# arkworks-rs/accumulation

Measured on NVIDIA B200. Metric: Pallas MSM Mpts/s @2^20, higher is better.
Workload: dtype u32x8 (255-bit Montgomery)

## Files before the change

accumulation_b200/csrc/accmsm.cu:

```cuda
#include <algorithm>
#include <chrono>
#include <cstdint>
#include <cstdio>
#include <cstdlib>
#include <cstring>
#include <functional>
#include <mutex>
#include <string>
#include <unordered_map>
#include <vector>

#include "../../include/accmsm.h"
#include "msm.cuh"
#include "sort.cuh"
#include "vec.cuh"
#include "ipa.cuh"
#include "wire.cuh"
#include "hostfp.hpp"

using namespace accmsm;

namespace {

enum Stage { ST_H2D = 0, ST_DIGITS, ST_SCAN, ST_SCATTER, ST_ACCUMULATE, ST_FIXUP, ST_REDUCE, ST_FINISH, ST_D2H, ST_VEC, ST_VEC_D2H, ST_COUNT };
// ... 30 lines not shown
void ipa_session_free(IpaSession *s);
struct CsrSet;
void csr_set_free(CsrSet *c);

struct GroupWorker;
struct GroupKey;
struct GroupCsr;

struct accmsm_ctx {
    std::vector<accmsm_ctx *> kids;
    std::vector<GroupWorker *> workers;
    std::unordered_map<uint64_t, GroupKey *> gkeys;
    std::unordered_map<uint64_t, GroupCsr *> gcsrs;
    std::unordered_map<uint64_t, struct GroupIpaSession *> gsessions;
    std::vector<char> peer_ok;
    std::vector<char> peer_read;
    void *d_gather = nullptr;
    size_t min_shard = size_t(1) << 16;
    int device = 0;
    int sm_count = 0;
    cudaStream_t stream = nullptr;
    std::mutex mu;
    std::string last_error;
    std::unordered_map<uint64_t, Bases> bases;
    std::unordered_map<uint64_t, struct IpaSession *> ipa_sessions;
    std::vector<struct IpaSession *> ipa_free;
    std::unordered_map<uint64_t, struct CsrSet *> csr_sets;
    std::vector<std::pair<void *, size_t>> vec_cache;
    uint64_t next_handle = 1;
    int window_bits = 0;
    uint64_t launches = 0;
    int acc_ctas_per_sm[2] = {0, 0};

    DevBuf<uint32_t> digits, hist, offsets, cursor, entries, cta_ids, tile_sums, tile_offs;
    DevBuf<xyzz_t> buckets, red_sum[2], red_wsum[2], cta_parts, partial;
    DevBuf<uint8_t> scalars, misc;
    DevBuf<uint2> sort_pairs;
    DevBuf<uint32_t> sort_tile_count, sort_part_count, sort_part_offs;
    int segments_override = 0;
    int seg0_pct = 25;
    std::vector<int> seg_pcts;
    bool no_coop_precompute = false;
    bool trace = false;
    std::vector<std::pair<std::string, cudaEvent_t>> trace_ev;
    std::vector<double> trace_host_us;
    int sort_lb_override = 0;
    DevBuf<uint8_t> oneshot_inf, ipa_tabs;
    bool no_ipa_tabs = false;
    bool no_coop_finish = false;
    DevBuf<affine_t> oneshot_xy, pair_pts[2];
    DevBuf<uint32_t> pair_off[2];
    DevBuf<uint8_t> pair_pref, pair_kinds, pair_tfac, pair_ctot, pair_cfac;
    int affine_rounds_override = -1;
    DevBuf<xyzz_t> fold_partial;
    DevBuf<uint32_t> fold_flag;
    int ipa_fold_rounds = 5, ipa_fold_min_log = 11;
    int fk_small_c = 0;
    xyzz_t *d_out_raw = nullptr;
    int out_curve = 0;
    uint64_t *h_out = nullptr;
    void *h_stage = nullptr;
    size_t stage_cap = 0;
    cudaEvent_t stage_done = nullptr;
    bool stage_busy = false;
    std::vector<cudaEvent_t> chunk_events;
    cudaStream_t copy_stream = nullptr;
    cudaStream_t aux_stream = nullptr;
    cudaEvent_t aux_fork = nullptr, aux_join = nullptr;
// ... 148 lines not shown
            *storage_cap = records;
        }
        table = *storage;
    } else {
        CU(ctx, cudaMalloc(&table, records * sizeof(affine_t)));
    }
    if (B.n <= PRECOMPUTE_COOP_MAX && !ctx->no_coop_precompute) {
        uint32_t groups = (uint32_t)((B.n + 31) / 32);
        if (B.curve == 0) k_precompute_coop<0><<<groups, 128, 0, ctx->stream>>>(B.d_xy, (uint32_t)B.n, c, nwin, table);
        else k_precompute_coop<1><<<groups, 128, 0, ctx->stream>>>(B.d_xy, (uint32_t)B.n, c, nwin, table);
    } else {
        uint32_t blocks = (uint32_t)((B.n + 127) / 128);
        if (B.curve == 0) k_precompute<0><<<blocks, 128, 0, ctx->stream>>>(B.d_xy, (uint32_t)B.n, c, nwin, table);
        else k_precompute<1><<<blocks, 128, 0, ctx->stream>>>(B.d_xy, (uint32_t)B.n, c, nwin, table);
    }
    ctx->launches++;
    if (!storage) {
        cudaError_t e = cudaStreamSynchronize(ctx->stream);
        if (e != cudaSuccess) { cudaFree(table); CU(ctx, e); }
    }
    B.d_table = table; B.pre_c = c; B.pre_nwin = nwin;
    return ACCMSM_OK;
}

bool use_table(const accmsm_ctx *ctx, const Bases &B, size_t n) {
    (void)n;
    if (!B.d_table) return false;
    return !ctx->window_bits || (uint32_t)ctx->window_bits == B.pre_c;
}

constexpr uint32_t ACC_WARP_MAX_KEYS = 8192;
constexpr size_t ACC_WARP_MAX_ENTRIES = 1u << 17;

#ifndef RED_L0_BLK
#define RED_L0_BLK 32
#endif

struct MsmJobs {
    uint32_t njobs = 1;
    size_t offset[MAX_JOBS] = {0};
    uint32_t tail_base = NONE_ID;
    uint32_t map_log_h = NONE_ID;
    MsmJobs() {}
    explicit MsmJobs(size_t off) { offset[0] = off; }
};

MsmShape make_shape(const accmsm_ctx *ctx, const Bases &B, const MsmJobs &jobs, size_t n, size_t n_for_c) {
    MsmShape sh;
    sh.n = (uint32_t)n;
    sh.njobs = jobs.njobs;
    sh.tail_base = jobs.tail_base;
    sh.map_log_h = jobs.map_log_h;
    for (int j = 0; j < MAX_JOBS; j++) sh.job_off[j] = j < (int)jobs.njobs ? (uint32_t)jobs.offset[j] : 0u;
    if (use_table(ctx, B, n)) {
        sh.c = B.pre_c;
        sh.nwin = B.pre_nwin;
        sh.nb = 1u << (sh.c - 1);
        sh.sets_per_job = 1;
        sh.hist_stride = 0;
        sh.ent_stride = (uint32_t)B.n;
    } else {
        sh.c = pick_window_bits(ctx, n_for_c);
        sh.nwin = (256 + sh.c - 1) / sh.c;
        sh.nb = 1u << (sh.c - 1);
        sh.sets_per_job = sh.nwin;
        sh.hist_stride = sh.nb;
        sh.ent_stride = 0;
    }
    sh.nkeys = sh.njobs * sh.sets_per_job * sh.nb;
    return sh;
// ... 107 lines not shown
        mark(ctx, ST_FIXUP, st);
    } else {
        const uint32_t *acc_offsets = ctx->offsets.p, *acc_entries = ctx->entries.p;
        const affine_t *acc_points = points;
        size_t acc_bound = n_entries;
        int rounds = into ? 0 : affine_rounds(ctx, sh, n_entries);
        for (int r = 0; r < rounds; r++) {
            const size_t out_bound = (acc_bound + sh.nkeys) / 2 + 1;
            CU(ctx, ctx->pair_off[r & 1].ensure(sh.nkeys + 1));
            CU(ctx, ctx->pair_pts[r & 1].ensure(out_bound));
            k_pair_counts<<<(sh.nkeys + 255) / 256, 256, 0, st>>>(acc_offsets, sh.nkeys, ctx->hist.p);
            ctx->launches++;
            { int src2 = launch_scan(ctx, ctx->hist.p, sh.nkeys, ctx->pair_off[r & 1].p, nullptr, st); if (src2) return src2; }
            uint32_t pgrid = (uint32_t)((out_bound + (size_t)PAIR_THREADS * PAIR_B - 1) / ((size_t)PAIR_THREADS * PAIR_B));
            CU(ctx, ctx->pair_pref.ensure(out_bound * 32));
            CU(ctx, ctx->pair_kinds.ensure(out_bound));
            CU(ctx, ctx->pair_tfac.ensure((size_t)pgrid * PAIR_THREADS * 32));
            CU(ctx, ctx->pair_ctot.ensure((size_t)pgrid * 32));
            CU(ctx, ctx->pair_cfac.ensure((size_t)pgrid * 32));
            const uint32_t *oin = acc_offsets, *oout = ctx->pair_off[r & 1].p;
            affine_t *pout = ctx->pair_pts[r & 1].p;
            if (r == 0) {
                k_pair_fwd<CURVE, true><<<pgrid, PAIR_THREADS, 0, st>>>(oin, oout, sh.nkeys, ctx->entries.p, points, ctx->pair_pref.p, ctx->pair_kinds.p, ctx->pair_tfac.p, ctx->pair_ctot.p);
                k_pair_mid<CURVE><<<1, PAIR_MID_THREADS, 0, st>>>(oout, sh.nkeys, ctx->pair_ctot.p, ctx->pair_cfac.p);
                k_pair_bwd<CURVE, true><<<pgrid, PAIR_THREADS, 0, st>>>(oin, oout, sh.nkeys, ctx->entries.p, points, ctx->pair_pref.p, ctx->pair_kinds.p, ctx->pair_tfac.p, ctx->pair_cfac.p, pout);
            } else {
                k_pair_fwd<CURVE, false><<<pgrid, PAIR_THREADS, 0, st>>>(oin, oout, sh.nkeys, nullptr, acc_points, ctx->pair_pref.p, ctx->pair_kinds.p, ctx->pair_tfac.p, ctx->pair_ctot.p);
                k_pair_mid<CURVE><<<1, PAIR_MID_THREADS, 0, st>>>(oout, sh.nkeys, ctx->pair_ctot.p, ctx->pair_cfac.p);
                k_pair_bwd<CURVE, false><<<pgrid, PAIR_THREADS, 0, st>>>(oin, oout, sh.nkeys, nullptr, acc_points, ctx->pair_pref.p, ctx->pair_kinds.p, ctx->pair_tfac.p, ctx->pair_cfac.p, pout);
            }
            ctx->launches += 3;
            acc_offsets = ctx->pair_off[r & 1].p; acc_entries = nullptr; acc_points = ctx->pair_pts[r & 1].p; acc_bound = out_bound;
        }
        int per_sm = ctx->acc_ctas_per_sm[CURVE];
        uint32_t gmax = (uint32_t)(ctx->sm_count * per_sm);
        uint32_t want = (uint32_t)((acc_bound + (size_t)ACC_THREADS * 8 - 1) / ((size_t)ACC_THREADS * 8));
        uint32_t grid = std::max(1u, std::min(gmax, want));
        CU(ctx, ctx->cta_ids.ensure(2 * grid));
        CU(ctx, ctx->cta_parts.ensure(2 * grid));
        size_t smem = 2 * ACC_THREADS * (sizeof(xyzz_t) + sizeof(uint32_t));
        if (into) k_accumulate<CURVE, true><<<grid, ACC_THREADS, smem, st>>>(acc_offsets, sh.nkeys, acc_entries, acc_points, ctx->buckets.p,
                                                                              ctx->cta_ids.p, ctx->cta_parts.p);
        else k_accumulate<CURVE, false><<<grid, ACC_THREADS, smem, st>>>(acc_offsets, sh.nkeys, acc_entries, acc_points, ctx->buckets.p,
                                                                          ctx->cta_ids.p, ctx->cta_parts.p);
        mark(ctx, ST_FIXUP, st);
        trace_point(ctx, st, "  k_accumulate done");
        uint32_t ns = 2 * grid;
        if (ns > (uint32_t)(FIX_THREADS * FIX_PER_T)) return fail_arg(ctx, "msm: accumulate grid exceeds the fix-up kernel's slots");
        size_t smem2 = ns * (sizeof(xyzz_t) + sizeof(uint32_t));
        cudaStream_t fx = fixup_aside ? aux_begin(ctx, st) : st;
        k_fixup<CURVE><<<1, FIX_THREADS, smem2, fx>>>(ctx->cta_ids.p, ctx->cta_parts.p, ns, ctx->buckets.p);
        ctx->launches += 2;
    }
    return ACCMSM_OK;
}

template <int CURVE>
int msm_reduce(accmsm_ctx *ctx, const MsmShape &sh, bool use_offsets, const xyzz_t *d_extra, uint32_t n_extra, xyzz_t *d_partial,
               bool normalise, cudaStream_t st, xyzz_t *d_out_raw) {
    if (!d_out_raw) d_out_raw = ctx->d_out_raw;
    ctx->out_curve = CURVE;
    const uint32_t nsets = sh.njobs * sh.sets_per_job;
    const uint32_t *offs = use_offsets ? ctx->offsets.p : nullptr;
    { int arc = aux_sync(ctx, st); if (arc) return arc; }
    mark(ctx, ST_REDUCE, st);
    const xyzz_t *window_sums = nullptr;
    {
        const uint32_t m = sh.c - 1, N0 = sh.nb;
        const uint32_t C0 = N0 > 1024 ? 1u << (m / 2) : 0, R0 = N0 > 1024 ? N0 / C0 : 0;
        CU(ctx, ctx->red_sum[0].ensure((size_t)nsets * (R0 + C0) + 1));
        CU(ctx, ctx->red_wsum[0].ensure((size_t)nsets * 128));
        CU(ctx, ctx->red_wsum[1].ensure(nsets));
        xyzz_t *scratch = ctx->red_sum[0].p, *leaf = ctx->red_wsum[0].p, *sums = ctx->red_wsum[1].p;
        CU(ctx, cudaMemsetAsync(leaf, 0, (size_t)nsets * 128 * sizeof(xyzz_t), st));
        int nlevels;
        SumTasks t1; memset(&t1, 0, sizeof t1);
        if (N0 > 1024) {
            SumTasks t0; memset(&t0, 0, sizeof t0);
            const bool split = (R0 + C0) * nsets > 320u && R0 > C0;
            const uint32_t CW = split ? 2 * C0 : C0;
            CU(ctx, ctx->red_sum[0].ensure((size_t)nsets * (R0 + CW) + 1));
            scratch = ctx->red_sum[0].p;
            t0.t[0] = SumTask{0, 0, R0, C0, C0, 1, 1, 0};
            if (split) {
                t0.ntasks = 3;
                t0.t[1] = SumTask{0, R0, C0, R0 / 2, 1, C0, 2, 0};
                t0.t[2] = SumTask{(R0 / 2) * C0, R0 + 1, C0, R0 / 2, 1, C0, 2, 0};
            } else {
                t0.ntasks = 2;
                t0.t[1] = SumTask{0, R0, C0, R0, 1, C0, 1, 0};
            }
            const uint32_t nout0 = R0 + (split ? 2 * C0 : C0);
            if (!split && (R0 + C0) * nsets <= 320u)
                k_sums_coop<CURVE><<<dim3(nout0, nsets), 128, 0, st>>>(ctx->buckets.p, N0, offs, scratch, R0 + CW, t0);
            else
                k_sums<CURVE, RED_L0_BLK><<<dim3(nout0, nsets), RED_L0_BLK, 0, st>>>(ctx->buckets.p, N0, offs, scratch, R0 + CW, t0);
            t1.ntasks = 4;
            const uint32_t pw = split ? 2u : 1u, pr = split ? 1u : 0u;
            t1.t[0] = SumTask{0, 0, R0 / 32, 32, 32, 1, 1, 0};            t1.t[1] = SumTask{0, 32, 32, R0 / 32, 1, 32, 1, 0};
            t1.t[2] = SumTask{R0, 64, C0 / 32, 32, 32 * pw, pw, 1, pr};   t1.t[3] = SumTask{R0, 96, 32, C0 / 32, pw, 32 * pw, 1, pr};
            k_sums_coop<CURVE><<<dim3(R0 / 32 + C0 / 32 + 64, nsets), 128, 0, st>>>(scratch, R0 + CW, nullptr, leaf, 128, t1);
            ctx->launches += 2;
            nlevels = 2;
        } else if (N0 > 32) {
            t1.ntasks = 2;
            t1.t[0] = SumTask{0, 0, N0 / 32, 32, 32, 1, 1, 0};     t1.t[1] = SumTask{0, 32, 32, N0 / 32, 1, 32, 1, 0};
            k_sums_coop<CURVE><<<dim3(N0 / 32 + 32, nsets), 128, 0, st>>>(ctx->buckets.p, N0, offs, leaf, 128, t1);
            ctx->launches++;
            nlevels = 1;
        } else {
            t1.ntasks = 1;
            t1.t[0] = SumTask{0, 0, N0, 1, 1, 1, 1, 0};
            k_sums_coop<CURVE><<<dim3(N0, nsets), 128, 0, st>>>(ctx->buckets.p, N0, offs, leaf, 128, t1);
            ctx->launches++;
            nlevels = 0;
        }
        uint32_t s0 = 0;
        while (C0 && (1u << s0) < C0) s0++;
        CU(ctx, ctx->red_sum[1].ensure((size_t)nsets * 5));
        const uint32_t narr = nlevels == 2 ? 4 : nlevels == 1 ? 2 : 1;
        k_leaf_scan_coop<CURVE><<<dim3(narr, nsets), 128, 0, st>>>(leaf, 128, ctx->red_sum[1].p);
        k_leaf_combine_coop<CURVE><<<nsets, 256, 0, st>>>(ctx->red_sum[1].p, nlevels, s0, sums);
        ctx->launches += 2;
        window_sums = sums;
    }
    mark(ctx, ST_FINISH, st);
    if (sh.sets_per_job > 1 && !ctx->no_coop_finish)
        k_finish_coop<CURVE><<<sh.njobs, 128, 0, st>>>(window_sums, sh.sets_per_job, sh.c, d_extra, n_extra, d_partial, normalise ? d_out_raw : nullptr);
    else
// ... 345 lines not shown
const char *accmsm_last_error(accmsm_ctx *ctx) { return ctx ? ctx->last_error.c_str() : "null ctx"; }

const char *accmsm_stage_name(int stage) { return stage >= 0 && stage < ST_COUNT ? STAGE_NAMES[stage] : ""; }

int accmsm_init(accmsm_ctx **out, int device) {
    if (!out) return ACCMSM_E_ARG;
    *out = nullptr;
    int count = 0;
    if (cudaGetDeviceCount(&count) != cudaSuccess || count == 0 || device < 0 || device >= count) return ACCMSM_E_CUDA;
    if (cudaSetDevice(device) != cudaSuccess) return ACCMSM_E_CUDA;
    accmsm_ctx *ctx = new accmsm_ctx();
    ctx->device = device;
    if (const char *e = getenv("ACCMSM_AFFINE_ROUNDS")) ctx->affine_rounds_override = atoi(e);
    if (const char *e = getenv("ACCMSM_SORT_LB")) ctx->sort_lb_override = atoi(e);
    if (const char *e = getenv("ACCMSM_SEGMENTS")) ctx->segments_override = atoi(e);
    if (const char *e = getenv("ACCMSM_SEG0_PCT")) ctx->seg0_pct = std::min(90, std::max(1, atoi(e)));
    if (const char *e = getenv("ACCMSM_SEG_PCTS")) { for (const char *q = e; *q;) { ctx->seg_pcts.push_back(atoi(q)); while (*q && *q != ',') q++; if (*q) q++; } }
    if (const char *e = getenv("ACCMSM_TRACE")) ctx->trace = atoi(e) != 0;
    if (const char *e = getenv("ACCMSM_NO_AUX")) ctx->no_aux = atoi(e) != 0;
    if (const char *e = getenv("ACCMSM_NO_IPA_TABS")) ctx->no_ipa_tabs = atoi(e) != 0;
    if (const char *e = getenv("ACCMSM_NO_COOP_FINISH")) ctx->no_coop_finish = atoi(e) != 0;
    if (const char *e = getenv("ACCMSM_NO_COOP_PRECOMPUTE")) ctx->no_coop_precompute = atoi(e) != 0;
    if (const char *e = getenv("ACCMSM_FK_C")) ctx->fk_small_c = atoi(e);
    cudaDeviceProp prop;
    if (cudaGetDeviceProperties(&prop, device) != cudaSuccess) { delete ctx; return ACCMSM_E_CUDA; }
    ctx->sm_count = prop.multiProcessorCount;
    if (cudaStreamCreateWithFlags(&ctx->stream, cudaStreamNonBlocking) != cudaSuccess) { delete ctx; return ACCMSM_E_CUDA; }
    for (int i = 0; i <= ST_COUNT; i++) { cudaEventCreate(&ctx->ev[i]); ctx->ev_valid[i] = false; }
    cudaEventCreateWithFlags(&ctx->stage_done, cudaEventDisableTiming);
    cudaEventCreateWithFlags(&ctx->ws_done, cudaEventDisableTiming);
    for (int i = 0; i < accmsm_ctx::ARG_SLOTS; i++) cudaEventCreateWithFlags(&ctx->arg_done[i], cudaEventDisableTiming);
    bool ok = cudaMallocHost(&ctx->h_args, accmsm_ctx::ARG_SLOTS * accmsm_ctx::ARG_SLOT_BYTES) == cudaSuccess && cudaMalloc(&ctx->d_out_raw, MAX_JOBS * sizeof(xyzz_t)) == cudaSuccess &&
              cudaMallocHost(&ctx->h_out, (MAX_JOBS * 16 + 64) * sizeof(uint64_t)) == cudaSuccess;
    size_t smem = 2 * ACC_THREADS * (sizeof(xyzz_t) + sizeof(uint32_t));
    size_t smem_fix = (size_t)FIX_THREADS * FIX_PER_T * (sizeof(xyzz_t) + sizeof(uint32_t));
    ok = ok && cudaFuncSetAttribute(k_accumulate<0, false>, cudaFuncAttributeMaxDynamicSharedMemorySize, (int)smem) == cudaSuccess;
    ok = ok && cudaFuncSetAttribute(k_accumulate<1, false>, cudaFuncAttributeMaxDynamicSharedMemorySize, (int)smem) == cudaSuccess;
    ok = ok && cudaFuncSetAttribute(k_accumulate<0, true>, cudaFuncAttributeMaxDynamicSharedMemorySize, (int)smem) == cudaSuccess;
    ok = ok && cudaFuncSetAttribute(k_accumulate<1, true>, cudaFuncAttributeMaxDynamicSharedMemorySize, (int)smem) == cudaSuccess;
    ok = ok && sort_opt_in<MemScalars<0>>() && sort_opt_in<MemScalars<1>>() && sort_opt_in<IpaScalars<0>>() && sort_opt_in<IpaScalars<1>>() &&
         sort_opt_in<IpaRoundScalars<0>>() && sort_opt_in<IpaRoundScalars<1>>() &&
         cudaFuncSetAttribute(k_sort_buckets, cudaFuncAttributeMaxDynamicSharedMemorySize, (int)SORT_SMEM_OPT_IN) == cudaSuccess;
    {
        const int tv = 2 * VEC_MAX_INPUTS * TVEC_THREADS * (int)sizeof(fe_t);
        ok = ok && cudaFuncSetAttribute(k_tvecs<0>, cudaFuncAttributeMaxDynamicSharedMemorySize, tv) == cudaSuccess &&
             cudaFuncSetAttribute(k_tvecs<1>, cudaFuncAttributeMaxDynamicSharedMemorySize, tv) == cudaSuccess;
    }
    ok = ok && cudaFuncSetAttribute(k_fixup<0>, cudaFuncAttributeMaxDynamicSharedMemorySize, (int)std::min<size_t>(smem_fix, 227 * 1024)) == cudaSuccess;
    ok = ok && cudaFuncSetAttribute(k_fixup<1>, cudaFuncAttributeMaxDynamicSharedMemorySize, (int)std::min<size_t>(smem_fix, 227 * 1024)) == cudaSuccess;
    if (ok) {
        cudaOccupancyMaxActiveBlocksPerMultiprocessor(&ctx->acc_ctas_per_sm[0], k_accumulate<0, false>, ACC_THREADS, smem);
        cudaOccupancyMaxActiveBlocksPerMultiprocessor(&ctx->acc_ctas_per_sm[1], k_accumulate<1, false>, ACC_THREADS, smem);
        for (int c = 0; c < 2; c++) {
            if (ctx->acc_ctas_per_sm[c] < 1) ctx->acc_ctas_per_sm[c] = 1;
            int cap = (FIX_THREADS * FIX_PER_T / 2) / ctx->sm_count;
            if (ctx->acc_ctas_per_sm[c] > cap) ctx->acc_ctas_per_sm[c] = std::max(1, cap);
        }
    }
    if (!ok) {
        ctx->last_error = cudaGetErrorString(cudaGetLastError());
        accmsm_destroy(ctx);
        return ACCMSM_E_CUDA;
    }
    *out = ctx;
    return ACCMSM_OK;
}

void accmsm_destroy(accmsm_ctx *ctx) {
    if (!ctx) return;
    if (is_group(ctx)) { group_destroy(ctx); return; }
    cudaSetDevice(ctx->device);
    if (ctx->stream) cudaStreamSynchronize(ctx->stream);
    for (auto &kv : ctx->bases) {
        cudaFree(kv.second.d_xy);
        if (kv.second.d_inf) cudaFree(kv.second.d_inf);
        if (kv.second.d_table) cudaFree(kv.second.d_table);
    }
    for (auto &kv : ctx->ipa_sessions) ipa_session_free(kv.second);
    for (auto *fs : ctx->ipa_free) ipa_session_free(fs);
    for (auto &kv : ctx->csr_sets) csr_set_free(kv.second);
    for (auto &b : ctx->vec_cache) cudaFree(b.first);
    ctx->digits.release(); ctx->hist.release(); ctx->offsets.release(); ctx->cursor.release(); ctx->entries.release();
    ctx->cta_ids.release(); ctx->tile_sums.release(); ctx->tile_offs.release(); ctx->buckets.release(); ctx->cta_parts.release(); ctx->partial.release();
    ctx->scalars.release(); ctx->misc.release(); ctx->oneshot_xy.release(); ctx->oneshot_inf.release(); ctx->ipa_tabs.release();
    ctx->sort_pairs.release(); ctx->sort_tile_count.release(); ctx->sort_part_count.release(); ctx->sort_part_offs.release();
    for (int i = 0; i < 2; i++) { ctx->pair_pts[i].release(); ctx->pair_off[i].release(); }
    ctx->fold_partial.release(); ctx->fold_flag.release();
    ctx->pair_pref.release(); ctx->pair_kinds.release(); ctx->pair_tfac.release(); ctx->pair_ctot.release(); ctx->pair_cfac.release();
    for (int i = 0; i < 2; i++) { ctx->red_sum[i].release(); ctx->red_wsum[i].release(); }
    if (ctx->d_out_raw) cudaFree(ctx->d_out_raw);
    if (ctx->h_out) cudaFreeHost(ctx->h_out);
    if (ctx->h_stage) cudaFreeHost(ctx->h_stage);
    if (ctx->stage_done) cudaEventDestroy(ctx->stage_done);
    if (ctx->ws_done) cudaEventDestroy(ctx->ws_done);
    for (int i = 0; i < accmsm_ctx::ARG_SLOTS; i++) if (ctx->arg_done[i]) cudaEventDestroy(ctx->arg_done[i]);
    if (ctx->h_args) cudaFreeHost(ctx->h_args);
    for (cudaEvent_t ev : ctx->chunk_events) cudaEventDestroy(ev);
    if (ctx->copy_stream) cudaStreamDestroy(ctx->copy_stream);
    if (ctx->aux_stream) cudaStreamDestroy(ctx->aux_stream);
    if (ctx->aux_fork) cudaEventDestroy(ctx->aux_fork);
    if (ctx->aux_join) cudaEventDestroy(ctx->aux_join);
    for (int i = 0; i <= ST_COUNT; i++) cudaEventDestroy(ctx->ev[i]);
    if (ctx->stream) cudaStreamDestroy(ctx->stream);
    delete ctx;
}

void *accmsm_host_alloc(size_t bytes) {
    void *p = nullptr;
    if (cudaMallocHost(&p, std::max<size_t>(bytes, 1)) != cudaSuccess) { (void)cudaGetLastError(); return nullptr; }
    return p;
}
void accmsm_host_free(void *p) { if (p) cudaFreeHost(p); }

int accmsm_set_window_bits(accmsm_ctx *ctx, int c) {
    if (!ctx || c < 0 || c > 16 || c == 1) return fail_arg(ctx, "window bits must be 0 (auto) or 2..16");
    for (accmsm_ctx *kid : ctx->kids) kid->window_bits = c;
// ... 415 lines not shown
```

accumulation_b200/csrc/msm.cuh:

```cuda
#pragma once
#include <cuda_runtime.h>
#include "ec.cuh"

namespace accmsm {

constexpr uint32_t NONE_ID = 0xffffffffu;
constexpr int ACC_THREADS = 256;
constexpr int FIX_THREADS = 512;
constexpr int FIX_PER_T = 3;
static_assert((size_t)FIX_THREADS * FIX_PER_T * (sizeof(uint32_t) + 128) <= 227 * 1024, "k_fixup slots must fit in one CTA's shared memory");
constexpr int MAX_WINDOWS = 64;
constexpr int MAX_JOBS = 8;

struct MsmShape {
    uint32_t n;
    uint32_t c;
    uint32_t nwin;
    uint32_t nb;
    uint32_t nkeys;
    uint32_t hist_stride;
    uint32_t ent_stride;
    uint32_t njobs;
    uint32_t sets_per_job;
    uint32_t job_off[MAX_JOBS];
    uint32_t tail_base;
    uint32_t map_log_h;
};
ACC_D uint32_t msm_base_index(const MsmShape &sh, uint32_t job, uint32_t i) {
    if (sh.tail_base != NONE_ID && i == sh.n - 1) return sh.tail_base;
    if (sh.map_log_h != NONE_ID) return sh.job_off[job] + ((i >> sh.map_log_h) << (sh.map_log_h + 1)) + (i & ((1u << sh.map_log_h) - 1u));
    return sh.job_off[job] + i;
}

ACC_D fe_t load_fe(const void *p) {
    const uint4 *q = reinterpret_cast<const uint4 *>(p);
    uint4 a = q[0], b = q[1];
    fe_t r;
    r.l[0] = a.x; r.l[1] = a.y; r.l[2] = a.z; r.l[3] = a.w; r.l[4] = b.x; r.l[5] = b.y; r.l[6] = b.z; r.l[7] = b.w;
    return r;
}
ACC_D fe_t load_fe_nc(const void *p) {
    const uint4 *q = reinterpret_cast<const uint4 *>(p);
    uint4 a = __ldg(q), b = __ldg(q + 1);
// ... 258 lines not shown
            uint32_t i = threadIdx.x + r * blockDim.x;
            any |= i < ns && i >= d && id[i] != NONE_ID && id[i] == id[i - d];
        }
        if (!__syncthreads_or(any)) break;
#pragma unroll 1
        for (int r = PER_T - 1; r >= 0; r--) {
            uint32_t i = threadIdx.x + r * blockDim.x;
            bool doit = i < ns && i >= d && id[i] != NONE_ID && id[i] == id[i - d];
            xyzz_t mine;
            if (doit) { mine = pt[i]; xyzz_t other = pt[i - d]; Cv::add(mine, other); }
            __syncthreads();
            if (doit) pt[i] = mine;
            __syncthreads();
        }
    }
}

ACC_D bool affine_is_identity_marker(const fe_t &x) {
    uint32_t d = 0xffffffffu;
#pragma unroll
    for (int i = 0; i < 8; i++) d &= x.l[i];
    return d == 0xffffffffu;
}
ACC_D affine_t affine_identity_marker() {
    affine_t r;
#pragma unroll
    for (int i = 0; i < 8; i++) { r.x.l[i] = 0xffffffffu; r.y.l[i] = 0u; }
    return r;
}
template <int CURVE, bool INTO>
__global__ void __launch_bounds__(ACC_THREADS, 2)
k_accumulate(const uint32_t *__restrict__ offsets, uint32_t nkeys, const uint32_t *__restrict__ entries,
             const affine_t *__restrict__ bases, xyzz_t *__restrict__ buckets,
             uint32_t *__restrict__ cta_ids, xyzz_t *__restrict__ cta_parts) {
    constexpr bool into = INTO;
    using Cv = Curve<CURVE>;
    extern __shared__ uint4 smem_raw[];
    xyzz_t *slot_pt = reinterpret_cast<xyzz_t *>(smem_raw);
    uint32_t *slot_id = reinterpret_cast<uint32_t *>(slot_pt + 2 * ACC_THREADS);

    const uint32_t M = offsets[nkeys];
    const uint32_t T = gridDim.x * blockDim.x;
    const uint32_t t = blockIdx.x * blockDim.x + threadIdx.x;
    const uint32_t L = (M + T - 1) / T;
    const uint64_t s64 = (uint64_t)t * L;
    const uint32_t s = s64 < M ? (uint32_t)s64 : M;
    const uint32_t e = (s64 + L < M) ? (uint32_t)(s64 + L) : M;

    uint32_t head_id = NONE_ID, tail_id = NONE_ID;
    slot_pt[2 * threadIdx.x + 1] = Cv::identity();
    if (s >= e) slot_pt[2 * threadIdx.x] = Cv::identity();

    if (s < e) {
        uint32_t lo = 0, hi = nkeys - 1;
        while (lo < hi) {
            uint32_t mid = (lo + hi) >> 1;
            if (offsets[mid + 1] > s) hi = mid; else lo = mid + 1;
        }
        uint32_t k = lo, bend = offsets[k + 1];
        bool first_run = true;
        xyzz_t acc = (into && s == offsets[k]) ? load_xyzz(buckets + k) : Cv::identity();
        uint32_t ent = entries ? entries[s] : s;
        affine_t pt = load_affine(bases + (ent & 0x7fffffffu));
#pragma unroll 1
        for (uint32_t p = s; p < e; p++) {
            if (p == bend) {
                if (first_run) { slot_pt[2 * threadIdx.x] = acc; head_id = k; first_run = false; }
                else store_xyzz(buckets + k, acc);
                acc = Cv::identity();
                k++; bend = offsets[k + 1];
                if (bend == p) {
                    uint32_t blo = k + 1, bhi = nkeys - 1;
                    while (blo < bhi) {
                        uint32_t mid = (blo + bhi) >> 1;
                        if (offsets[mid + 1] > p) bhi = mid; else blo = mid + 1;
                    }
                    k = blo; bend = offsets[k + 1];
                }
                if (into) acc = load_xyzz(buckets + k);
            }
            const uint32_t cur_sign = ent >> 31;
            affine_t cur = pt;
            if (p + 1 < e) {
                ent = entries ? entries[p + 1] : p + 1;
                pt = load_affine(bases + (ent & 0x7fffffffu));
            }
            if (cur_sign) cur.y = Cv::F::neg(cur.y);
            if (entries || !affine_is_identity_marker(cur.x)) Cv::madd(acc, cur);
        }
        if (first_run) { slot_pt[2 * threadIdx.x] = acc; head_id = k; tail_id = k; }
        else { slot_pt[2 * threadIdx.x + 1] = acc; tail_id = k; }
    }
    slot_id[2 * threadIdx.x] = head_id;
    slot_id[2 * threadIdx.x + 1] = tail_id;
    __syncthreads();
    const uint32_t ns = 2 * ACC_THREADS;
    seg_scan<CURVE, 2>(slot_pt, slot_id, ns);

    const uint32_t first_id = slot_id[0];
    __shared__ uint32_t last_id_s;
    if (threadIdx.x == 0) last_id_s = NONE_ID;
    __syncthreads();
    for (int r = 0; r < 2; r++) {
        uint32_t i = threadIdx.x + r * blockDim.x;
        bool valid = slot_id[i] != NONE_ID;
        bool next_valid = (i + 1 < ns) && slot_id[i + 1] != NONE_ID;
        if (valid && !next_valid) last_id_s = slot_id[i];
    }
    __syncthreads();
    const uint32_t last_id = last_id_s;
    if (threadIdx.x == 0) {
        cta_ids[2 * blockIdx.x] = first_id;
        cta_ids[2 * blockIdx.x + 1] = last_id;
        if (first_id == last_id) store_xyzz(cta_parts + 2 * blockIdx.x + 1, Cv::identity());
    }
    for (int r = 0; r < 2; r++) {
        uint32_t i = threadIdx.x + r * blockDim.x;
        uint32_t id = slot_id[i];
        if (id == NONE_ID) continue;
        bool group_end = (i + 1 == ns) || slot_id[i + 1] != id;
        if (!group_end) continue;
        if (id == first_id) store_xyzz(cta_parts + 2 * blockIdx.x, slot_pt[i]);
        else if (id == last_id) store_xyzz(cta_parts + 2 * blockIdx.x + 1, slot_pt[i]);
        else store_xyzz(buckets + id, slot_pt[i]);
    }
}

template <int CURVE>
__global__ void __launch_bounds__(128) k_accumulate_warp_coop(const uint32_t *__restrict__ offsets, uint32_t nkeys,
                                                               const uint32_t *__restrict__ entries,
                                                               const affine_t *__restrict__ bases, xyzz_t *__restrict__ buckets);

constexpr int PAIR_THREADS = 256;
constexpr int PAIR_B = 32;
constexpr int PAIR_MID_THREADS = 1024;

__global__ void __launch_bounds__(256) k_pair_counts(const uint32_t *__restrict__ offsets, uint32_t nkeys,
                                                      uint32_t *__restrict__ counts) {
    uint32_t k = blockIdx.x * blockDim.x + threadIdx.x;
    if (k < nkeys) counts[k] = (offsets[k + 1] - offsets[k] + 1u) >> 1;
}

template <bool FIRST>
ACC_D fe_t pair_load_x(const uint32_t *__restrict__ entries, const affine_t *__restrict__ pts, uint32_t i) {
    return load_fe_nc(&pts[FIRST ? (entries[i] & 0x7fffffffu) : i].x);
}
template <int CURVE, bool FIRST>
ACC_D fe_t pair_load_y(const uint32_t *__restrict__ entries, const affine_t *__restrict__ pts, uint32_t i) {
    using F = typename Curve<CURVE>::F;
    if (FIRST) {
        uint32_t ent = entries[i];
        fe_t y = load_fe_nc(&pts[ent & 0x7fffffffu].y);
        return (ent >> 31) ? F::neg(y) : y;
    }
    return load_fe_nc(&pts[i].y);
}
enum : uint8_t { PAIR_PASS0 = 0, PAIR_PASS1 = 1, PAIR_ADD = 2, PAIR_DBL = 3, PAIR_IDENT = 4 };

// ... 158 lines not shown
        k = w.k; bstart = off_out[k];
    }
#pragma unroll 1
    for (uint32_t s = s1; s-- > s0;) {
        if (s < bstart) {
            k--; bstart = off_out[k];
            if (s < bstart) { PairWalk w; w.init(off_out, nkeys, s); k = w.k; bstart = off_out[k]; }
        }
        const uint32_t i0 = off_in[k] + 2 * (s - bstart);
        const uint8_t kind = kinds[s];
        affine_t r;
        if (kind == PAIR_PASS0 || kind == PAIR_PASS1) {
            const uint32_t i = kind == PAIR_PASS0 ? i0 : i0 + 1;
            r.x = pair_load_x<FIRST>(entries, pts_in, i);
            r.y = pair_load_y<CURVE, FIRST>(entries, pts_in, i);
        } else if (kind == PAIR_IDENT) {
            r = affine_identity_marker();
        } else {
            const fe_t x0 = pair_load_x<FIRST>(entries, pts_in, i0), y0 = pair_load_y<CURVE, FIRST>(entries, pts_in, i0);
            const fe_t x1 = pair_load_x<FIRST>(entries, pts_in, i0 + 1);
            fe_t den, num;
            if (kind == PAIR_ADD) { den = F::sub(x1, x0); num = F::sub(pair_load_y<CURVE, FIRST>(entries, pts_in, i0 + 1), y0); }
            else { den = F::dbl(y0); fe_t xx = F::sqr(x0); num = F::add(F::dbl(xx), xx); }
            const fe_t dinv = F::mul(rinv, load_fe(pref + (size_t)s * 32));
            rinv = F::mul(rinv, den);
            const fe_t lam = F::mul(num, dinv);
            r.x = F::sub(F::sub(F::sqr(lam), x0), x1);
            r.y = F::sub(F::mul(lam, F::sub(x0, r.x)), y0);
        }
        store_fe(&pts_out[s].x, r.x); store_fe(&pts_out[s].y, r.y);
    }
}

template <int CURVE>
__global__ void __launch_bounds__(FIX_THREADS) k_fixup(const uint32_t *__restrict__ cta_ids,
                                                 const xyzz_t *__restrict__ cta_parts, uint32_t ns,
                                                 xyzz_t *__restrict__ buckets) {
    extern __shared__ uint4 smem_raw[];
    xyzz_t *slot_pt = reinterpret_cast<xyzz_t *>(smem_raw);
    uint32_t *slot_id = reinterpret_cast<uint32_t *>(slot_pt + ns);
    for (uint32_t i = threadIdx.x; i < ns; i += blockDim.x) {
        slot_id[i] = cta_ids[i];
        slot_pt[i] = load_xyzz(cta_parts + i);
    }
    __syncthreads();
    seg_scan<CURVE, FIX_PER_T, FpCall>(slot_pt, slot_id, ns);
    for (uint32_t i = threadIdx.x; i < ns; i += blockDim.x) {
        uint32_t id = slot_id[i];
        if (id == NONE_ID) continue;
        bool group_end = (i + 1 == ns) || slot_id[i + 1] != id;
        if (group_end) store_xyzz(buckets + id, slot_pt[i]);
    }
}


struct SumTask {
    uint32_t in_off;
    uint32_t out_off;
    uint32_t n_out;
    uint32_t len;
    uint32_t stride_out;
    uint32_t stride_len;
    uint32_t out_stride;
    uint32_t pair;
};
struct SumTasks {
    SumTask t[4];
    uint32_t ntasks;
};

template <int CURVE, int BLK>
__global__ void __launch_bounds__(BLK) k_sums(const xyzz_t *__restrict__ in, uint32_t in_set_stride,
                                              const uint32_t *__restrict__ offsets, xyzz_t *__restrict__ out,
                                              uint32_t out_set_stride, SumTasks tasks) {
    using Cv = Curve<CURVE, FpCall>;
    __shared__ xyzz_t part[BLK / 32];
    uint32_t o = blockIdx.x, ti = 0;
    while (ti + 1 < tasks.ntasks && o >= tasks.t[ti].n_out) { o -= tasks.t[ti].n_out; ti++; }
    const SumTask tk = tasks.t[ti];
    const uint32_t set = blockIdx.y;
    const xyzz_t *src = in + (size_t)set * in_set_stride;
    const uint32_t *offs = offsets ? offsets + (size_t)set * in_set_stride : nullptr;
    xyzz_t acc = Cv::identity();
    for (uint32_t j = threadIdx.x; j < tk.len; j += BLK) {
        uint32_t idx = tk.in_off + o * tk.stride_out + j * tk.stride_len;
        if (!offs || offs[idx + 1] != offs[idx]) { xyzz_t b = load_xyzz(src + idx); Cv::add(acc, b); }
        if (tk.pair) { xyzz_t b = load_xyzz(src + idx + 1); Cv::add(acc, b); }
    }
    const uint32_t lane = threadIdx.x & 31, wid = threadIdx.x >> 5;
    const uint32_t live = tk.len < BLK ? tk.len : BLK;
#pragma unroll 1
    for (int d = 16; d >= 1; d >>= 1) {
        if ((uint32_t)d < live) {
            xyzz_t other = shfl_down_xyzz(acc, d);
            if (lane < (uint32_t)d) Cv::add(acc, other);
        }
    }
    if (BLK > 32) {
        if (lane == 0) part[wid] = acc;
        __syncthreads();
        if (wid == 0) {
            acc = lane < BLK / 32 && lane * 32 < live ? part[lane] : Cv::identity();
#pragma unroll 1
            for (int d = BLK / 64; d >= 1; d >>= 1) {
                if ((uint32_t)d * 32 < live) {
                    xyzz_t other = shfl_down_xyzz(acc, d);
                    if (lane < (uint32_t)d) Cv::add(acc, other);
                }
            }
        }
    }
    if (threadIdx.x == 0) store_xyzz(out + (size_t)set * out_set_stride + tk.out_off + o * (tk.out_stride ? tk.out_stride : 1u), acc);
}


template <int CURVE>
__global__ void __launch_bounds__(128) k_accumulate_warp_coop(const uint32_t *__restrict__ offsets, uint32_t nkeys,
                                                               const uint32_t *__restrict__ entries,
                                                               const affine_t *__restrict__ bases, xyzz_t *__restrict__ buckets) {
    using Cv = Curve<CURVE, FpCall>;
    using Co = Coop<CURVE>;
    __shared__ CoopScratch scratch;
    const uint32_t k = blockIdx.x, lane = threadIdx.x & 31;
    CoopCtx c{&scratch, threadIdx.x >> 5, lane, 1, 0};
    const uint32_t b0 = offsets[k], b1 = offsets[k + 1];
    if (b0 == b1) return;
    xyzz_t acc = Cv::identity();
#pragma unroll 1
    for (uint32_t p0 = b0; p0 < b1; p0 += 32) {
        const uint32_t p = p0 + lane;
        xyzz_t q = Cv::identity();
        if (p < b1) {
            uint32_t ent = entries[p];
            affine_t pt = load_affine(bases + (ent & 0x7fffffffu));
            if (ent >> 31) pt.y = Cv::F::neg(pt.y);
            q = Cv::from_affine(pt);
        }
        if (p0 == b0) acc = q; else Co::add(c, acc, q);
    }
    const uint32_t m = b1 - b0;
#pragma unroll 1
    for (int d = 16; d >= 1; d >>= 1) {
        if ((uint32_t)d < m) {
            xyzz_t other = shfl_down_xyzz(acc, d), t = acc;
            if (lane >= (uint32_t)d) other = Cv::identity();
// ... 275 lines not shown
```

Baseline: 359.3.

## Replace in-CTA carry scan and single-block fixup with global slot merge kernel

k_accumulate no longer runs a shared-memory segmented scan per CTA. Each thread writes its head and tail partial buckets straight to global slot arrays. A new multi-block k_merge kernel does the segmented scans over those slots, and the last block to finish (found with an atomic counter) resolves the cross-block carries in chunks. This removes the dynamic shared memory and the block-wide scan from the hot accumulate kernel, and drops the cap on accumulate occupancy that the single-CTA fixup imposed. In exchange, much more slot data goes through global memory. Separately, the level-0 bucket sums switch to a k_sums_tree kernel that gives each output one warp, packs two outputs per block, and reduces through a shared-memory tree instead of xyzz shuffles.

```diff
diff --git a/accumulation_b200/csrc/accmsm.cu b/accumulation_b200/csrc/accmsm.cu
--- a/accumulation_b200/csrc/accmsm.cu
+++ b/accumulation_b200/csrc/accmsm.cu
@@ -86,8 +86,9 @@
     uint64_t launches = 0;
     int acc_ctas_per_sm[2] = {0, 0};
 
-    DevBuf<uint32_t> digits, hist, offsets, cursor, entries, cta_ids, tile_sums, tile_offs;
-    DevBuf<xyzz_t> buckets, red_sum[2], red_wsum[2], cta_parts, partial;
+    DevBuf<uint32_t> digits, hist, offsets, cursor, entries, slot_ids, tile_sums, tile_offs;
+    DevBuf<xyzz_t> buckets, red_sum[2], red_wsum[2], slot_pts, partial;
+    DevBuf<uint32_t> merge_done;
     DevBuf<uint8_t> scalars, misc;
     DevBuf<uint2> sort_pairs;
     DevBuf<uint32_t> sort_tile_count, sort_part_count, sort_part_offs;
@@ -302,10 +303,6 @@
 constexpr uint32_t ACC_WARP_MAX_KEYS = 8192;
 constexpr size_t ACC_WARP_MAX_ENTRIES = 1u << 17;
 
-#ifndef RED_L0_BLK
-#define RED_L0_BLK 32
-#endif
-
 struct MsmJobs {
     uint32_t njobs = 1;
     size_t offset[MAX_JOBS] = {0};
@@ -479,25 +476,28 @@
             ctx->launches += 3;
             acc_offsets = ctx->pair_off[r & 1].p; acc_entries = nullptr; acc_points = ctx->pair_pts[r & 1].p; acc_bound = out_bound;
         }
-        int per_sm = ctx->acc_ctas_per_sm[CURVE];
-        uint32_t gmax = (uint32_t)(ctx->sm_count * per_sm);
+        uint32_t gmax = (uint32_t)(ctx->sm_count * ctx->acc_ctas_per_sm[CURVE]);
         uint32_t want = (uint32_t)((acc_bound + (size_t)ACC_THREADS * 8 - 1) / ((size_t)ACC_THREADS * 8));
         uint32_t grid = std::max(1u, std::min(gmax, want));
-        CU(ctx, ctx->cta_ids.ensure(2 * grid));
-        CU(ctx, ctx->cta_parts.ensure(2 * grid));
-        size_t smem = 2 * ACC_THREADS * (sizeof(xyzz_t) + sizeof(uint32_t));
-        if (into) k_accumulate<CURVE, true><<<grid, ACC_THREADS, smem, st>>>(acc_offsets, sh.nkeys, acc_entries, acc_points, ctx->buckets.p,
-                                                                              ctx->cta_ids.p, ctx->cta_parts.p);
-        else k_accumulate<CURVE, false><<<grid, ACC_THREADS, smem, st>>>(acc_offsets, sh.nkeys, acc_entries, acc_points, ctx->buckets.p,
-                                                                          ctx->cta_ids.p, ctx->cta_parts.p);
+        const uint32_t ns = 2 * grid * ACC_THREADS;
+        const uint32_t mgrid = (ns + MERGE_THREADS - 1) / MERGE_THREADS;
+        CU(ctx, ctx->slot_ids.ensure(ns + 2 * mgrid));
+        CU(ctx, ctx->slot_pts.ensure(ns + 2 * mgrid));
+        if (!ctx->merge_done.p) {
+            CU(ctx, ctx->merge_done.ensure(1));
+            CU(ctx, cudaMemsetAsync(ctx->merge_done.p, 0, sizeof(uint32_t), st));
+        }
+        if (into) k_accumulate<CURVE, true><<<grid, ACC_THREADS, 0, st>>>(acc_offsets, sh.nkeys, acc_entries, acc_points, ctx->buckets.p,
+                                                                           ctx->slot_ids.p, ctx->slot_pts.p);
+        else k_accumulate<CURVE, false><<<grid, ACC_THREADS, 0, st>>>(acc_offsets, sh.nkeys, acc_entries, acc_points, ctx->buckets.p,
+                                                                       ctx->slot_ids.p, ctx->slot_pts.p);
+        ctx->launches++;
         mark(ctx, ST_FIXUP, st);
         trace_point(ctx, st, "  k_accumulate done");
-        uint32_t ns = 2 * grid;
-        if (ns > (uint32_t)(FIX_THREADS * FIX_PER_T)) return fail_arg(ctx, "msm: accumulate grid exceeds the fix-up kernel's slots");
-        size_t smem2 = ns * (sizeof(xyzz_t) + sizeof(uint32_t));
         cudaStream_t fx = fixup_aside ? aux_begin(ctx, st) : st;
-        k_fixup<CURVE><<<1, FIX_THREADS, smem2, fx>>>(ctx->cta_ids.p, ctx->cta_parts.p, ns, ctx->buckets.p);
-        ctx->launches += 2;
+        k_merge<CURVE><<<mgrid, MERGE_THREADS, MERGE_SMEM, fx>>>(ctx->slot_ids.p, ctx->slot_pts.p, ns, ctx->slot_ids.p + ns, ctx->slot_pts.p + ns,
+                                                                  ctx->merge_done.p, ctx->buckets.p);
+        ctx->launches++;
     }
     return ACCMSM_OK;
 }
@@ -541,7 +541,8 @@
             if (!split && (R0 + C0) * nsets <= 320u)
                 k_sums_coop<CURVE><<<dim3(nout0, nsets), 128, 0, st>>>(ctx->buckets.p, N0, offs, scratch, R0 + CW, t0);
             else
-                k_sums<CURVE, RED_L0_BLK><<<dim3(nout0, nsets), RED_L0_BLK, 0, st>>>(ctx->buckets.p, N0, offs, scratch, R0 + CW, t0);
+                k_sums_tree<CURVE><<<dim3((nout0 + SUMS_TREE_WARPS - 1) / SUMS_TREE_WARPS, nsets), SUMS_TREE_WARPS * 32, 0, st>>>(
+                    ctx->buckets.p, N0, offs, scratch, R0 + CW, t0, nout0);
             t1.ntasks = 4;
             const uint32_t pw = split ? 2u : 1u, pr = split ? 1u : 0u;
             t1.t[0] = SumTask{0, 0, R0 / 32, 32, 32, 1, 1, 0};            t1.t[1] = SumTask{0, 32, 32, R0 / 32, 1, 32, 1, 0};
@@ -953,12 +954,6 @@
     for (int i = 0; i < accmsm_ctx::ARG_SLOTS; i++) cudaEventCreateWithFlags(&ctx->arg_done[i], cudaEventDisableTiming);
     bool ok = cudaMallocHost(&ctx->h_args, accmsm_ctx::ARG_SLOTS * accmsm_ctx::ARG_SLOT_BYTES) == cudaSuccess && cudaMalloc(&ctx->d_out_raw, MAX_JOBS * sizeof(xyzz_t)) == cudaSuccess &&
               cudaMallocHost(&ctx->h_out, (MAX_JOBS * 16 + 64) * sizeof(uint64_t)) == cudaSuccess;
-    size_t smem = 2 * ACC_THREADS * (sizeof(xyzz_t) + sizeof(uint32_t));
-    size_t smem_fix = (size_t)FIX_THREADS * FIX_PER_T * (sizeof(xyzz_t) + sizeof(uint32_t));
-    ok = ok && cudaFuncSetAttribute(k_accumulate<0, false>, cudaFuncAttributeMaxDynamicSharedMemorySize, (int)smem) == cudaSuccess;
-    ok = ok && cudaFuncSetAttribute(k_accumulate<1, false>, cudaFuncAttributeMaxDynamicSharedMemorySize, (int)smem) == cudaSuccess;
-    ok = ok && cudaFuncSetAttribute(k_accumulate<0, true>, cudaFuncAttributeMaxDynamicSharedMemorySize, (int)smem) == cudaSuccess;
-    ok = ok && cudaFuncSetAttribute(k_accumulate<1, true>, cudaFuncAttributeMaxDynamicSharedMemorySize, (int)smem) == cudaSuccess;
     ok = ok && sort_opt_in<MemScalars<0>>() && sort_opt_in<MemScalars<1>>() && sort_opt_in<IpaScalars<0>>() && sort_opt_in<IpaScalars<1>>() &&
          sort_opt_in<IpaRoundScalars<0>>() && sort_opt_in<IpaRoundScalars<1>>() &&
          cudaFuncSetAttribute(k_sort_buckets, cudaFuncAttributeMaxDynamicSharedMemorySize, (int)SORT_SMEM_OPT_IN) == cudaSuccess;
@@ -967,16 +962,12 @@
         ok = ok && cudaFuncSetAttribute(k_tvecs<0>, cudaFuncAttributeMaxDynamicSharedMemorySize, tv) == cudaSuccess &&
              cudaFuncSetAttribute(k_tvecs<1>, cudaFuncAttributeMaxDynamicSharedMemorySize, tv) == cudaSuccess;
     }
-    ok = ok && cudaFuncSetAttribute(k_fixup<0>, cudaFuncAttributeMaxDynamicSharedMemorySize, (int)std::min<size_t>(smem_fix, 227 * 1024)) == cudaSuccess;
-    ok = ok && cudaFuncSetAttribute(k_fixup<1>, cudaFuncAttributeMaxDynamicSharedMemorySize, (int)std::min<size_t>(smem_fix, 227 * 1024)) == cudaSuccess;
+    ok = ok && cudaFuncSetAttribute(k_merge<0>, cudaFuncAttributeMaxDynamicSharedMemorySize, (int)MERGE_SMEM) == cudaSuccess &&
+         cudaFuncSetAttribute(k_merge<1>, cudaFuncAttributeMaxDynamicSharedMemorySize, (int)MERGE_SMEM) == cudaSuccess;
     if (ok) {
-        cudaOccupancyMaxActiveBlocksPerMultiprocessor(&ctx->acc_ctas_per_sm[0], k_accumulate<0, false>, ACC_THREADS, smem);
-        cudaOccupancyMaxActiveBlocksPerMultiprocessor(&ctx->acc_ctas_per_sm[1], k_accumulate<1, false>, ACC_THREADS, smem);
-        for (int c = 0; c < 2; c++) {
-            if (ctx->acc_ctas_per_sm[c] < 1) ctx->acc_ctas_per_sm[c] = 1;
-            int cap = (FIX_THREADS * FIX_PER_T / 2) / ctx->sm_count;
-            if (ctx->acc_ctas_per_sm[c] > cap) ctx->acc_ctas_per_sm[c] = std::max(1, cap);
-        }
+        cudaOccupancyMaxActiveBlocksPerMultiprocessor(&ctx->acc_ctas_per_sm[0], k_accumulate<0, false>, ACC_THREADS, 0);
+        cudaOccupancyMaxActiveBlocksPerMultiprocessor(&ctx->acc_ctas_per_sm[1], k_accumulate<1, false>, ACC_THREADS, 0);
+        for (int c = 0; c < 2; c++) ctx->acc_ctas_per_sm[c] = std::max(1, ctx->acc_ctas_per_sm[c]);
     }
     if (!ok) {
         ctx->last_error = cudaGetErrorString(cudaGetLastError());
@@ -1002,7 +993,7 @@
     for (auto &kv : ctx->csr_sets) csr_set_free(kv.second);
     for (auto &b : ctx->vec_cache) cudaFree(b.first);
     ctx->digits.release(); ctx->hist.release(); ctx->offsets.release(); ctx->cursor.release(); ctx->entries.release();
-    ctx->cta_ids.release(); ctx->tile_sums.release(); ctx->tile_offs.release(); ctx->buckets.release(); ctx->cta_parts.release(); ctx->partial.release();
+    ctx->slot_ids.release(); ctx->merge_done.release(); ctx->tile_sums.release(); ctx->tile_offs.release(); ctx->buckets.release(); ctx->slot_pts.release(); ctx->partial.release();
     ctx->scalars.release(); ctx->misc.release(); ctx->oneshot_xy.release(); ctx->oneshot_inf.release(); ctx->ipa_tabs.release();
     ctx->sort_pairs.release(); ctx->sort_tile_count.release(); ctx->sort_part_count.release(); ctx->sort_part_offs.release();
     for (int i = 0; i < 2; i++) { ctx->pair_pts[i].release(); ctx->pair_off[i].release(); }
diff --git a/accumulation_b200/csrc/msm.cuh b/accumulation_b200/csrc/msm.cuh
--- a/accumulation_b200/csrc/msm.cuh
+++ b/accumulation_b200/csrc/msm.cuh
@@ -6,9 +6,6 @@
 
 constexpr uint32_t NONE_ID = 0xffffffffu;
 constexpr int ACC_THREADS = 256;
-constexpr int FIX_THREADS = 512;
-constexpr int FIX_PER_T = 3;
-static_assert((size_t)FIX_THREADS * FIX_PER_T * (sizeof(uint32_t) + 128) <= 227 * 1024, "k_fixup slots must fit in one CTA's shared memory");
 constexpr int MAX_WINDOWS = 64;
 constexpr int MAX_JOBS = 8;
 
@@ -333,13 +330,9 @@
 __global__ void __launch_bounds__(ACC_THREADS, 2)
 k_accumulate(const uint32_t *__restrict__ offsets, uint32_t nkeys, const uint32_t *__restrict__ entries,
              const affine_t *__restrict__ bases, xyzz_t *__restrict__ buckets,
-             uint32_t *__restrict__ cta_ids, xyzz_t *__restrict__ cta_parts) {
+             uint32_t *__restrict__ slot_ids, xyzz_t *__restrict__ slot_pts) {
     constexpr bool into = INTO;
     using Cv = Curve<CURVE>;
-    extern __shared__ uint4 smem_raw[];
-    xyzz_t *slot_pt = reinterpret_cast<xyzz_t *>(smem_raw);
-    uint32_t *slot_id = reinterpret_cast<uint32_t *>(slot_pt + 2 * ACC_THREADS);
-
     const uint32_t M = offsets[nkeys];
     const uint32_t T = gridDim.x * blockDim.x;
     const uint32_t t = blockIdx.x * blockDim.x + threadIdx.x;
@@ -349,9 +342,6 @@
     const uint32_t e = (s64 + L < M) ? (uint32_t)(s64 + L) : M;
 
     uint32_t head_id = NONE_ID, tail_id = NONE_ID;
-    slot_pt[2 * threadIdx.x + 1] = Cv::identity();
-    if (s >= e) slot_pt[2 * threadIdx.x] = Cv::identity();
-
     if (s < e) {
         uint32_t lo = 0, hi = nkeys - 1;
         while (lo < hi) {
@@ -366,7 +356,7 @@
 #pragma unroll 1
         for (uint32_t p = s; p < e; p++) {
             if (p == bend) {
-                if (first_run) { slot_pt[2 * threadIdx.x] = acc; head_id = k; first_run = false; }
+                if (first_run) { store_xyzz(slot_pts + 2 * t, acc); head_id = k; first_run = false; }
                 else store_xyzz(buckets + k, acc);
                 acc = Cv::identity();
                 k++; bend = offsets[k + 1];
@@ -389,42 +379,11 @@
             if (cur_sign) cur.y = Cv::F::neg(cur.y);
             if (entries || !affine_is_identity_marker(cur.x)) Cv::madd(acc, cur);
         }
-        if (first_run) { slot_pt[2 * threadIdx.x] = acc; head_id = k; tail_id = k; }
-        else { slot_pt[2 * threadIdx.x + 1] = acc; tail_id = k; }
-    }
-    slot_id[2 * threadIdx.x] = head_id;
-    slot_id[2 * threadIdx.x + 1] = tail_id;
-    __syncthreads();
-    const uint32_t ns = 2 * ACC_THREADS;
-    seg_scan<CURVE, 2>(slot_pt, slot_id, ns);
-
-    const uint32_t first_id = slot_id[0];
-    __shared__ uint32_t last_id_s;
-    if (threadIdx.x == 0) last_id_s = NONE_ID;
-    __syncthreads();
-    for (int r = 0; r < 2; r++) {
-        uint32_t i = threadIdx.x + r * blockDim.x;
-        bool valid = slot_id[i] != NONE_ID;
-        bool next_valid = (i + 1 < ns) && slot_id[i + 1] != NONE_ID;
-        if (valid && !next_valid) last_id_s = slot_id[i];
-    }
-    __syncthreads();
-    const uint32_t last_id = last_id_s;
-    if (threadIdx.x == 0) {
-        cta_ids[2 * blockIdx.x] = first_id;
-        cta_ids[2 * blockIdx.x + 1] = last_id;
-        if (first_id == last_id) store_xyzz(cta_parts + 2 * blockIdx.x + 1, Cv::identity());
-    }
-    for (int r = 0; r < 2; r++) {
-        uint32_t i = threadIdx.x + r * blockDim.x;
-        uint32_t id = slot_id[i];
-        if (id == NONE_ID) continue;
-        bool group_end = (i + 1 == ns) || slot_id[i + 1] != id;
-        if (!group_end) continue;
-        if (id == first_id) store_xyzz(cta_parts + 2 * blockIdx.x, slot_pt[i]);
-        else if (id == last_id) store_xyzz(cta_parts + 2 * blockIdx.x + 1, slot_pt[i]);
-        else store_xyzz(buckets + id, slot_pt[i]);
-    }
+        if (first_run) { store_xyzz(slot_pts + 2 * t, acc); store_xyzz(slot_pts + 2 * t + 1, Cv::identity()); head_id = k; }
+        else store_xyzz(slot_pts + 2 * t + 1, acc);
+        tail_id = k;
+    }
+    reinterpret_cast<uint2 *>(slot_ids)[t] = make_uint2(head_id, tail_id);
 }
 
 template <int CURVE>
@@ -649,25 +608,70 @@
     }
 }
 
-template <int CURVE>
-__global__ void __launch_bounds__(FIX_THREADS) k_fixup(const uint32_t *__restrict__ cta_ids,
-                                                 const xyzz_t *__restrict__ cta_parts, uint32_t ns,
-                                                 xyzz_t *__restrict__ buckets) {
+constexpr int MERGE_THREADS = 512;
+constexpr size_t MERGE_SMEM = (size_t)MERGE_THREADS * (sizeof(xyzz_t) + sizeof(uint32_t));
+ACC_D xyzz_t load_xyzz_cg(const xyzz_t *p) {
+    const uint4 *q = reinterpret_cast<const uint4 *>(p);
+    xyzz_t r;
+    uint32_t *w = reinterpret_cast<uint32_t *>(&r);
+#pragma unroll
+    for (int i = 0; i < 8; i++) { uint4 v = __ldcg(q + i); w[4 * i] = v.x; w[4 * i + 1] = v.y; w[4 * i + 2] = v.z; w[4 * i + 3] = v.w; }
+    return r;
+}
+template <int CURVE>
+__global__ void __launch_bounds__(MERGE_THREADS) k_merge(const uint32_t *__restrict__ ids, const xyzz_t *__restrict__ pts, uint32_t n,
+                                                         uint32_t *carry_ids, xyzz_t *carry_pts, uint32_t *done,
+                                                         xyzz_t *__restrict__ dst) {
+    using Cv = Curve<CURVE, FpCall>;
     extern __shared__ uint4 smem_raw[];
     xyzz_t *slot_pt = reinterpret_cast<xyzz_t *>(smem_raw);
-    uint32_t *slot_id = reinterpret_cast<uint32_t *>(slot_pt + ns);
-    for (uint32_t i = threadIdx.x; i < ns; i += blockDim.x) {
-        slot_id[i] = cta_ids[i];
-        slot_pt[i] = load_xyzz(cta_parts + i);
-    }
-    __syncthreads();
-    seg_scan<CURVE, FIX_PER_T, FpCall>(slot_pt, slot_id, ns);
-    for (uint32_t i = threadIdx.x; i < ns; i += blockDim.x) {
-        uint32_t id = slot_id[i];
-        if (id == NONE_ID) continue;
-        bool group_end = (i + 1 == ns) || slot_id[i + 1] != id;
-        if (group_end) store_xyzz(buckets + id, slot_pt[i]);
-    }
+    uint32_t *slot_id = reinterpret_cast<uint32_t *>(slot_pt + MERGE_THREADS);
+    __shared__ uint32_t last_id_s;
+    __shared__ bool is_last_s;
+    const uint32_t tid = threadIdx.x, b = blockIdx.x, base = b * MERGE_THREADS;
+    const uint32_t ns = n - base < (uint32_t)MERGE_THREADS ? n - base : (uint32_t)MERGE_THREADS;
+    if (tid < ns) { slot_id[tid] = ids[base + tid]; slot_pt[tid] = load_xyzz(pts + base + tid); }
+    if (tid == 0) last_id_s = NONE_ID;
+    __syncthreads();
+    seg_scan<CURVE, 1, FpCall>(slot_pt, slot_id, ns);
+    if (tid < ns && slot_id[tid] != NONE_ID && (tid + 1 == ns || slot_id[tid + 1] == NONE_ID)) last_id_s = slot_id[tid];
+    __syncthreads();
+    const uint32_t first_id = slot_id[0], last_id = last_id_s;
+    if (tid == 0) {
+        carry_ids[2 * b] = first_id;
+        carry_ids[2 * b + 1] = last_id;
+        if (first_id == NONE_ID) store_xyzz(carry_pts + 2 * b, Cv::identity());
+        if (first_id == last_id) store_xyzz(carry_pts + 2 * b + 1, Cv::identity());
+    }
+    if (tid < ns && slot_id[tid] != NONE_ID && (tid + 1 == ns || slot_id[tid + 1] != slot_id[tid])) {
+        const uint32_t id = slot_id[tid];
+        xyzz_t *to = id == first_id ? carry_pts + 2 * b
+                   : id == last_id ? carry_pts + 2 * b + 1
+                   : dst + id;
+        store_xyzz(to, slot_pt[tid]);
+    }
+    __threadfence();
+    __syncthreads();
+    if (tid == 0) is_last_s = atomicAdd(done, 1u) == gridDim.x - 1;
+    __syncthreads();
+    if (!is_last_s) return;
+    __threadfence();
+    const uint32_t n2 = 2 * gridDim.x;
+    if (tid == 0) { slot_id[0] = NONE_ID; slot_pt[0] = Cv::identity(); }
+#pragma unroll 1
+    for (uint32_t c0 = 0; c0 < n2; c0 += MERGE_THREADS - 1) {
+        const uint32_t m = n2 - c0 < (uint32_t)MERGE_THREADS - 1 ? n2 - c0 : (uint32_t)MERGE_THREADS - 1;
+        const bool final_round = c0 + m == n2;
+        if (tid < m) { slot_id[tid + 1] = __ldcg(carry_ids + c0 + tid); slot_pt[tid + 1] = load_xyzz_cg(carry_pts + c0 + tid); }
+        __syncthreads();
+        seg_scan<CURVE, 1, FpCall>(slot_pt, slot_id, m + 1);
+        const uint32_t id = tid <= m ? slot_id[tid] : NONE_ID;
+        if (id != NONE_ID && (tid == m ? final_round : slot_id[tid + 1] != id)) store_xyzz(dst + id, slot_pt[tid]);
+        __syncthreads();
+        if (tid == 0 && !final_round) { slot_id[0] = slot_id[m]; slot_pt[0] = slot_pt[m]; }
+        __syncthreads();
+    }
+    if (tid == 0) *done = 0u;
 }
 
 
@@ -686,48 +690,43 @@
     uint32_t ntasks;
 };
 
-template <int CURVE, int BLK>
-__global__ void __launch_bounds__(BLK) k_sums(const xyzz_t *__restrict__ in, uint32_t in_set_stride,
-                                              const uint32_t *__restrict__ offsets, xyzz_t *__restrict__ out,
-                                              uint32_t out_set_stride, SumTasks tasks) {
+constexpr int SUMS_TREE_WARPS = 2;
+template <int CURVE, int NW = SUMS_TREE_WARPS>
+__global__ void __launch_bounds__(NW * 32) k_sums_tree(const xyzz_t *__restrict__ in, uint32_t in_set_stride,
+                                                             const uint32_t *__restrict__ offsets, xyzz_t *__restrict__ out,
+                                                             uint32_t out_set_stride, SumTasks tasks, uint32_t nout) {
     using Cv = Curve<CURVE, FpCall>;
-    __shared__ xyzz_t part[BLK / 32];
-    uint32_t o = blockIdx.x, ti = 0;
+    __shared__ xyzz_t part[NW * 32];
+    const uint32_t lane = threadIdx.x & 31, wid = threadIdx.x >> 5;
+    uint32_t o = blockIdx.x * NW + wid, ti = 0;
+    const bool live = o < nout;
     while (ti + 1 < tasks.ntasks && o >= tasks.t[ti].n_out) { o -= tasks.t[ti].n_out; ti++; }
     const SumTask tk = tasks.t[ti];
     const uint32_t set = blockIdx.y;
     const xyzz_t *src = in + (size_t)set * in_set_stride;
     const uint32_t *offs = offsets ? offsets + (size_t)set * in_set_stride : nullptr;
     xyzz_t acc = Cv::identity();
-    for (uint32_t j = threadIdx.x; j < tk.len; j += BLK) {
-        uint32_t idx = tk.in_off + o * tk.stride_out + j * tk.stride_len;
-        if (!offs || offs[idx + 1] != offs[idx]) { xyzz_t b = load_xyzz(src + idx); Cv::add(acc, b); }
-        if (tk.pair) { xyzz_t b = load_xyzz(src + idx + 1); Cv::add(acc, b); }
-    }
-    const uint32_t lane = threadIdx.x & 31, wid = threadIdx.x >> 5;
-    const uint32_t live = tk.len < BLK ? tk.len : BLK;
-#pragma unroll 1
-    for (int d = 16; d >= 1; d >>= 1) {
-        if ((uint32_t)d < live) {
-            xyzz_t other = shfl_down_xyzz(acc, d);
-            if (lane < (uint32_t)d) Cv::add(acc, other);
-        }
-    }
-    if (BLK > 32) {
-        if (lane == 0) part[wid] = acc;
-        __syncthreads();
-        if (wid == 0) {
-            acc = lane < BLK / 32 && lane * 32 < live ? part[lane] : Cv::identity();
-#pragma unroll 1
-            for (int d = BLK / 64; d >= 1; d >>= 1) {
-                if ((uint32_t)d * 32 < live) {
-                    xyzz_t other = shfl_down_xyzz(acc, d);
-                    if (lane < (uint32_t)d) Cv::add(acc, other);
-                }
-            }
-        }
-    }
-    if (threadIdx.x == 0) store_xyzz(out + (size_t)set * out_set_stride + tk.out_off + o * (tk.out_stride ? tk.out_stride : 1u), acc);
+    if (live) {
+#pragma unroll 1
+        for (uint32_t j = lane; j < tk.len; j += 32) {
+            uint32_t idx = tk.in_off + o * tk.stride_out + j * tk.stride_len;
+            if (!offs || offs[idx + 1] != offs[idx]) { xyzz_t b = load_xyzz(src + idx); Cv::add(acc, b); }
+            if (tk.pair) { xyzz_t b = load_xyzz(src + idx + 1); Cv::add(acc, b); }
+        }
+    }
+    part[threadIdx.x] = acc;
+    __syncthreads();
+#pragma unroll 1
+    for (uint32_t h = 16; h >= 1; h >>= 1) {
+        if (threadIdx.x < NW * h) {
+            const uint32_t q = (threadIdx.x / h) * 32 + threadIdx.x % h;
+            xyzz_t x = part[q], y = part[q + h];
+            Cv::add(x, y);
+            part[q] = x;
+        }
+        __syncthreads();
+    }
+    if (live && lane == 0) store_xyzz(out + (size_t)set * out_set_stride + tk.out_off + o * (tk.out_stride ? tk.out_stride : 1u), part[wid * 32]);
 }
 
 
```

New measurement: 358.8, median of 6. No clear change (-0.1%).
